# MECLabTUDA/Lifelong-nnUNet

Hardware: AMD Instinct MI355X
Metric: 3D patches/sec (whole node) + mean Dice vs ref, 5-level 3D Generic_UNet training step (higher is better)
Workload: dtype f16 (fp32 accumulate, fp32 master weights); 1 GPU; BASELINE configs[1]: nnUNetTrainerSequential.run_iteration, 160x192x160 patches, batch 2/GPU, num_pool 5, base 32, 3 logits; global_batch=2, parallelism=dp1, distinct_resident_batches=2, deterministic_wgrad=False

## Files before the change

lifelong-nnunet_amd/csrc/igemm_up2.hip:

```cpp
#include "igemm_common.h"

namespace {

constexpr int TZ = 2, TY = 8, TX = 8, PZ = 3, PY = 9, PX = 9;
constexpr int P = PZ * PY * PX;
constexpr int CK = 16, ROWB = 32, MB = 32;
constexpr int XBYTES = P * ROWB;
constexpr int XCHUNKS = P * 2;
constexpr int NT = 256;
constexpr int XN = (XCHUNKS + NT - 1) / NT;

template <int MODE>
struct UpCfg {
    static constexpr int NTAP = MODE == 0 ? 27 : 8;
    static constexpr int WBYTES = NTAP * MB * ROWB;
    static constexpr int WCHUNKS = NTAP * MB * 2;
    static constexpr int WN = (WCHUNKS + NT - 1) / NT;
};

__device__ __forceinline__ int up_xaddr(int pz, int py, int px, int c2) {
    return ((pz * PY + py) * PX + px) * ROWB + ((c2 ^ (py & 1)) << 4);
}
__device__ __forceinline__ int up_waddr(int row, int c2) { return row * ROWB + ((c2 ^ ((row >> 3) & 1)) << 4); }

__device__ __forceinline__ void up_lane_voxel(int v, int& r, int& x) {
    if (v < 4) { r = 0; x = v; }
    else if (v < 12) { r = 2; x = v - 4; }
    else if (v < 16) { r = 0; x = v - 8; }
    else if (v < 20) { r = 3; x = v - 16; }
    else if (v < 28) { r = 1; x = v - 20; }
    else { r = 3; x = v - 24; }
}

template <int MODE>
__global__ __launch_bounds__(NT, 2) void igemm_up2_kernel(const ConvParams p, int mblocks) {
    using Cfg = UpCfg<MODE>;
    constexpr int WN = Cfg::WN, WBYTES = Cfg::WBYTES, WCHUNKS = Cfg::WCHUNKS;
    extern __shared__ __attribute__((aligned(16))) char smem[];
    char* const xb = smem;
    char* const wb = smem + 2 * XBYTES;

    const int tid = threadIdx.x, lane = tid & 63, wave = tid >> 6;
    const int v = lane & 31, hk = lane >> 5;
    const int m0 = (blockIdx.x % mblocks) * MB;
    int t = blockIdx.x / mblocks;
    const int tx = t % p.tiles_x; t /= p.tiles_x;
    const int ty = t % p.tiles_y; t /= p.tiles_y;
    const int tz = t % p.tiles_z; t /= p.tiles_z;
    const int n = t, qz0 = tz * TZ, qy0 = ty * TY, qx0 = tx * TX;
    const int nchunks = (p.C + CK - 1) / CK;
    const bool interior = qz0 + PZ <= p.Di && qy0 + PY <= p.Hi && qx0 + PX <= p.Wi && (p.C % CK) == 0;

    int xrel[XN], xlds[XN];
#pragma unroll
    for (int i = 0; i < XN; ++i) {
        const int idx = min(i * NT + tid, XCHUNKS - 1);
        const int pos = idx >> 1, c2 = idx & 1;
        const int px = pos % PX, py = (pos / PX) % PY, pz = pos / (PX * PY);
        xrel[i] = ((pz * p.Hi + py) * p.Wi + px) * p.ld_x + c2 * 8;
        xlds[i] = up_xaddr(pz, py, px, c2);
    }
    int wrel[WN], wlds[WN];
#pragma unroll
    for (int i = 0; i < WN; ++i) {
        const int idx = min(i * NT + tid, WCHUNKS - 1);
        const int c2 = idx & 1, row = idx >> 1, r = row % MB, tl = row / MB;
        wrel[i] = (tl * MB + r) * 16 + c2 * 8;
        wlds[i] = up_waddr(row, c2);
    }

    half8 xr[XN], wr[WN];
    unsigned xok = 0;
    const half8 zero8 = {0, 0, 0, 0, 0, 0, 0, 0};
    const long xbase = ((((long)n * p.Di + qz0) * p.Hi + qy0) * p.Wi + qx0) * p.ld_x;
    const int nck16 = p.KCpad >> 4;
    const half_t* const wbase = p.wp + (long)(m0 >> 5) * nck16 * Cfg::NTAP * 512;

    auto load_x = [&](int c0) {
        if (interior) {
            const half_t* bp = p.x + xbase + c0;
#pragma unroll
            for (int i = 0; i < XN; ++i) xr[i] = *reinterpret_cast<const half8*>(bp + xrel[i]);
            xok = 0xFFFFu;
        } else {
            unsigned m = 0;
#pragma unroll
            for (int i = 0; i < XN; ++i) {
                const int idx = min(i * NT + tid, XCHUNKS - 1);
                const int pos = idx >> 1, c2 = idx & 1;
                const int px = pos % PX, py = (pos / PX) % PY, pz = pos / (PX * PY);
                const bool ok = qz0 + pz < p.Di && qy0 + py < p.Hi && qx0 + px < p.Wi && c0 + c2 * 8 < p.C;
                xr[i] = *reinterpret_cast<const half8*>(p.x + (ok ? xbase + c0 + xrel[i] : 0));
                m |= (ok ? 1u : 0u) << i;
            }
            xok = m;
        }
    };
    auto store_x = [&](char* buf) {
#pragma unroll
        for (int i = 0; i < XN; ++i)
            if (i * NT + tid < XCHUNKS) *reinterpret_cast<half8*>(buf + xlds[i]) = ((xok >> i) & 1u) ? xr[i] : zero8;
    };
    auto load_w = [&](int c0) {
#pragma unroll
        for (int i = 0; i < WN; ++i) wr[i] = *reinterpret_cast<const half8*>(wbase + (long)(c0 >> 4) * Cfg::NTAP * 512 + wrel[i]);
    };
    auto store_w = [&](char* buf) {
#pragma unroll
        for (int i = 0; i < WN; ++i)
            if (i * NT + tid < WCHUNKS) *reinterpret_cast<half8*>(buf + wlds[i]) = wr[i];
    };

    int vr, vx;
    up_lane_voxel(v, vr, vx);
    const int wz = wave >> 1, wy = (wave & 1) * 4 + vr;
    int lterm[2];
#pragma unroll
    for (int par = 0; par < 2; ++par) lterm[par] = ((wz * PY + wy) * PX + vx) * ROWB + ((hk ^ ((wy + par) & 1)) << 4);
    const int a_lane = v * ROWB + ((hk ^ ((v >> 3) & 1)) << 4);

    floatx16 acc[8];
#pragma unroll
    for (int c = 0; c < 8; ++c)
#pragma unroll
        for (int i = 0; i < 16; ++i) acc[c][i] = 0.f;

    load_x(0);
    load_w(0);
    store_x(xb);
    store_w(wb);
    __syncthreads();

#pragma unroll 1
    for (int ch = 0; ch < nchunks; ++ch) {
        const bool more = ch + 1 < nchunks;
        const char* xl = xb + (ch & 1) * XBYTES;
        const char* wl = wb + (ch & 1) * WBYTES;
        if (more) {
            load_x((ch + 1) * CK);
            load_w((ch + 1) * CK);
        }
        if (MODE == 0) {
            half8 fb[2][2][2];
#pragma unroll
            for (int oz = 0; oz < 2; ++oz)
#pragma unroll
                for (int oy = 0; oy < 2; ++oy)
#pragma unroll
                    for (int ox = 0; ox < 2; ++ox)
                        fb[oz][oy][ox] = *reinterpret_cast<const half8*>(xl + ((oz * PY + oy) * PX + ox) * ROWB + lterm[oy]);
#pragma unroll
            for (int cls = 0; cls < 8; ++cls) {
                const int pz = cls >> 2, py = (cls >> 1) & 1, px = cls & 1;
#pragma unroll
                for (int a = 0; a <= pz; ++a)
#pragma unroll
                    for (int b = 0; b <= py; ++b)
#pragma unroll
                        for (int c = 0; c <= px; ++c) {
                            const int dz = pz ? 2 * a : 1, dy = py ? 2 * b : 1, dx = px ? 2 * c : 1;
                            const int oz = pz ? 1 - a : 0, oy = py ? 1 - b : 0, ox = px ? 1 - c : 0;
                            const int slot = dz * 9 + dy * 3 + dx;
                            const half8 fa = *reinterpret_cast<const half8*>(wl + slot * MB * ROWB + a_lane);
                            acc[cls] = __builtin_amdgcn_mfma_f32_32x32x16_f16(fa, fb[oz][oy][ox], acc[cls], 0, 0, 0);
                        }
            }
        } else {
            const half8 fb = *reinterpret_cast<const half8*>(xl + lterm[0]);
#pragma unroll
            for (int cls = 0; cls < 8; ++cls) {
                const half8 fa = *reinterpret_cast<const half8*>(wl + cls * MB * ROWB + a_lane);
                acc[cls] = __builtin_amdgcn_mfma_f32_32x32x16_f16(fa, fb, acc[cls], 0, 0, 0);
            }
        }
        if (more) {
            store_x(xb + ((ch + 1) & 1) * XBYTES);
            store_w(wb + ((ch + 1) & 1) * WBYTES);
        }
        __syncthreads();
    }

    constexpr int RS = 1040;
    char* const stg = smem;
    const int qz = qz0 + wz, qy = qy0 + wy;
    const int skey = (vx >> 1) & 3;
    const int eox = (lane >> 2) & 15, ec = lane & 3;
    const int egx = 2 * qx0 + eox, em = m0 + ec * 8;
    auto out_ptr = [&](int pz, int rr) -> half8* {
        const int row = wave * 8 + rr, zl = row >> 4, oyl = row & 15;
        const int oz = 2 * (qz0 + zl) + pz, oy = 2 * qy0 + oyl;
        const bool ok = oz < p.Do && oy < p.Ho && egx < p.Wo && em < p.M;
        return ok ? reinterpret_cast<half8*>(p.y + ((((long)n * p.Do + oz) * p.Ho + oy) * p.Wo + egx) * p.ld_y + em) : nullptr;
    };
#pragma unroll
    for (int pz = 0; pz < 2; ++pz) {
        half8 olds[8];
        if (p.accumulate) {
#pragma unroll
            for (int rr = 0; rr < 8; ++rr) {
                const half8* d = out_ptr(pz, rr);
                olds[rr] = *(d ? d : reinterpret_cast<const half8*>(p.y));
            }
        }
#pragma unroll
        for (int c4 = 0; c4 < 4; ++c4) {
            const int cls = pz * 4 + c4, py = c4 >> 1, px = c4 & 1;
            char* vb = stg + (wz * 16 + 2 * wy + py) * RS + (2 * vx + px) * 64;
#pragma unroll
            for (int qq = 0; qq < 4; ++qq) {
                const half4 o = {(half_t)acc[cls][qq * 4 + 0], (half_t)acc[cls][qq * 4 + 1], (half_t)acc[cls][qq * 4 + 2],
                                 (half_t)acc[cls][qq * 4 + 3]};
                *reinterpret_cast<half4*>(vb + (((2 * qq + hk) ^ skey) << 3)) = o;
            }
        }
        __syncthreads();
        {
            const int rkey = (eox >> 2) & 3;
#pragma unroll
            for (int rr = 0; rr < 8; ++rr) {
                const int row = wave * 8 + rr;
                half8 v = *reinterpret_cast<const half8*>(stg + row * RS + eox * 64 + ((ec ^ (rkey >> 1)) << 4));
                if (rkey & 1) v = half8{v[4], v[5], v[6], v[7], v[0], v[1], v[2], v[3]};
                half8* dst = out_ptr(pz, rr);
                if (dst) {
                    if (p.accumulate) {
#pragma unroll
                        for (int e = 0; e < 8; ++e) v[e] = (half_t)((float)v[e] + (float)olds[rr][e]);
                    }
                    *dst = v;
                }
            }
        }
        if (pz == 0) __syncthreads();
    }
    (void)qz; (void)qy;
}

template <int MODE>
int launch_up2(hipStream_t s, ConvParams& p, const char* name) {
    using Cfg = UpCfg<MODE>;
    p.tiles_z = lnn_cdiv((p.Do + 1) / 2, TZ); p.tiles_y = lnn_cdiv((p.Ho + 1) / 2, TY); p.tiles_x = lnn_cdiv((p.Wo + 1) / 2, TX);
    const int mblocks = lnn_cdiv(p.M, MB);
    const long blocks = (long)p.N * p.tiles_z * p.tiles_y * p.tiles_x * mblocks;
    const size_t lds_main = 2 * XBYTES + 2 * Cfg::WBYTES, lds_stage = 32 * 1040;
    const size_t lds = lds_main > lds_stage ? lds_main : lds_stage;
    auto kern = igemm_up2_kernel<MODE>;
    static bool attr_set = false;
    if (!attr_set) {
        hipFuncSetAttribute(reinterpret_cast<const void*>(kern), hipFuncAttributeMaxDynamicSharedMemorySize, 80 * 1024);
        attr_set = true;
    }
    hipLaunchKernelGGL(kern, dim3((unsigned)blocks), dim3(NT), lds, s, p, mblocks);
    LNN_CHECK_LAUNCH(name);
    return LNN_OK;
}

}

int lnn_launch_up2_dgrad(hipStream_t s, ConvParams& p, const char* name) { return launch_up2<0>(s, p, name); }
int lnn_launch_up2_convT(hipStream_t s, ConvParams& p, const char* name) { return launch_up2<1>(s, p, name); }
```

lifelong-nnunet_amd/csrc/lnn_debug.h:

```cpp
#ifndef LNN_DEBUG_H
#define LNN_DEBUG_H
#include "../../include/lnn_hip.h"
#ifdef __cplusplus
extern "C" {
#endif

int lnn_debug_tr16_probe(lnn_stream_t s, float* out256);

int lnn_debug_set_phase_buffer(void* dev_ptr_6x_u64);
int lnn_debug_force_conv_kernel(int which);
int lnn_debug_force_down2_kernel(int which);
int lnn_debug_set_v9_zseg(int segments);

int lnn_debug_set_k133_v9(int mode);
int lnn_debug_last_k133_on_v9(void);

int lnn_debug_set_gen_mode(int mode);

int lnn_debug_last_dgrad_reduce_fused(void);

int lnn_debug_set_cu_budget(int cus);

#ifdef __cplusplus
}
#endif
#endif
```

lifelong-nnunet_amd/native.py:

```python
from __future__ import annotations

import ctypes as C
import os

_HERE = os.path.dirname(os.path.abspath(__file__))
LIB_PATH = os.environ.get("LNN_LIB_PATH") or os.path.join(_HERE, "csrc", "liblnn_hip.so")

_p = C.c_void_p
_i = C.c_int
_l = C.c_long
_f = C.c_float
_sz = C.c_size_t

SIGNATURES = {
    "lnn_last_error": (C.c_char_p, []),
    "lnn_version": (_i, []),
    "lnn_device_info": (_i, [C.POINTER(_i), C.POINTER(_i), C.c_char_p, _i]),
    "lnn_pack_weights": (_i, [_p, _p, _p, _i, _i, _i, _l, _l, _l]),
    "lnn_packed_weight_elems": (_sz, [_i, _i, _i]),
    "lnn_conv3d_fwd": (_i, [_p, _p, _i, _p, _p, _p, _i, _i, _i, _i, _i, _i, _i, _i]),
    "lnn_conv3d_dgrad": (_i, [_p, _p, _i, _p, _p, _i, _i, _i, _i, _i, _i, _i, _i, _i]),
    "lnn_conv3d_wgrad": (_i, [_p, _p, _i, _p, _i, _p, _i, _i, _i, _i, _i, _i, _i]),
    "lnn_conv3d_fwd_cat": (_i, [_p, _p, _p, _i, _i, _p, _p, _p, _i, _i, _i, _i, _i, _i, _i]),
    "lnn_conv3d_fwd_in_stats": (_i, [_p, _p, _p, _i, _i, _p, _p, _p, _i, _i, _i, _i, _i, _i, _i, _f, _p, _p, _p, _p, _l]),
    "lnn_conv3d_dgrad_ws": (_i, [_p, _p, _i, _p, _p, _i, _i, _i, _i, _i, _i, _i, _i, _i, _p, _l]),
    "lnn_conv3d_dgrad_cat": (_i, [_p, _p, _i, _p, _p, _p, _i, _i, _i, _i, _i, _i, _i, _i, _i]),
    "lnn_conv3d_dgrad_cat_ws": (_i, [_p, _p, _i, _p, _p, _p, _i, _i, _i, _i, _i, _i, _i, _i, _i, _p, _l]),
    "lnn_conv3d_wgrad_cat": (_i, [_p, _p, _p, _i, _i, _p, _i, _p, _i, _i, _i, _i, _i, _i]),
    "lnn_convT3d_k2s2_fwd": (_i, [_p, _p, _i, _p, _p, _i, _i, _i, _i, _i, _i, _i]),
    "lnn_convT3d_k2s2_dgrad": (_i, [_p, _p, _i, _p, _p, _i, _i, _i, _i, _i, _i, _i, _i]),
    "lnn_convT3d_k2s2_wgrad": (_i, [_p, _p, _i, _p, _i, _p, _i, _i, _i, _i, _i, _i]),
    "lnn_conv3d_wgrad_det": (_i, [_p, _p, _i, _p, _i, _p, _i, _i, _i, _i, _i, _i, _i, _p, _l]),
    "lnn_conv3d_wgrad_cat_det": (_i, [_p, _p, _p, _i, _i, _p, _i, _p, _i, _i, _i, _i, _i, _i, _p, _l]),
    "lnn_convT3d_k2s2_wgrad_det": (_i, [_p, _p, _i, _p, _i, _p, _i, _i, _i, _i, _i, _i, _p, _l]),
    "lnn_unpack_wgrad": (_i, [_p, _p, _p, _i, _i, _i, _l, _l, _l, _f, _i]),
    "lnn_pack_weights_batched": (_i, [_p, _p, _p, _p, _i, _l]),
    "lnn_unpack_wgrad_batched": (_i, [_p, _p, _p, _p, _i, _l, _f, _i]),
    "lnn_wgrad_panel_elems": (_sz, [_i, _i, _i]),
    "lnn_instnorm_stats": (_i, [_p, _p, _i, _l, _i, _f, _p, _p, _p]),
    "lnn_instnorm_lrelu_fwd": (_i, [_p, _p, _p, _i, _i, _l, _i, _p, _p, _p, _p, _f]),
    "lnn_instnorm_lrelu_seg_fwd": (_i, [_p, _p, _p, _i, _i, _l, _i, _p, _p, _p, _p, _f, _p, _p, _i]),
    "lnn_instnorm_lrelu_bwd": (_i, [_p, _p, _p, _i, _i, _l, _i, _p, _p, _p, _p, _f, _p, _p, _p, _f, _p]),
    "lnn_instnorm_ws_doubles": (_sz, [_i, _i]),
    "lnn_instnorm_lrelu_seg_bwd": (_i, [_p, _p, _p, _i, _p, _p, _p, _i, _i, _l, _i, _p, _p, _p, _p, _f, _p, _p, _f, _p]),
    "lnn_instnorm_lrelu_seg_bwd_ws_doubles": (_sz, [_i, _i]),
    "lnn_instnorm_lrelu_bwd_sums": (_i, [_p, _p, _p, _i, _i, _l, _i, _p, _p, _p, _p, _f, _p, _p, _f, _p]),
    "lnn_conv3d_dgrad_in_bwd_sums": (_i, [_p, _p, _i, _p, _p, _i, _i, _i, _i, _i, _i, _i, _p, _p, _p, _p, _p, _f, _p, _p, _f, _p, _p, _l]),
    "lnn_instnorm_lrelu_bwd_apply": (_i, [_p, _p, _p, _i, _i, _l, _i, _p, _p, _p, _p, _f, _p]),
    "lnn_instnorm_small_volume": (_i, []),
    "lnn_conv3d_fwd_in_lrelu": (_i, [_p, _p, _p, _i, _i, _p, _p, _p, _i, _i, _i, _i, _i, _i, _i, _f, _p, _p, _p, _p, _f, _p, _i, _p, _p, _l]),
    "lnn_conv3d_dgrad_in_bwd": (_i, [_p, _p, _i, _p, _p, _i, _i, _i, _i, _i, _i, _i, _p, _p, _p, _p, _p, _f, _p, _p, _f, _p, _p, _l]),
    "lnn_conv3d_wgrad_c1_in_bwd": (_i, [_p, _p, _p, _p, _i, _p, _i, _i, _i, _i, _i, _p, _p, _p, _p, _f, _p, _p, _l]),
    "lnn_seg1x1_fwd": (_i, [_p, _p, _i, _p, _p, _i, _l, _i, _i]),
    "lnn_seg1x1_bwd": (_i, [_p, _p, _i, _p, _p, _p, _i, _p, _i, _l, _i, _i, _i, _f, _p]),
    "lnn_seg1x1_bwd_ws_floats": (_sz, [_i, _i]),
    "lnn_dice_ce_fwd": (_i, [_p, _p, _p, _i, _i, _l, _i, _f, _p, _p]),
    "lnn_dice_ce_fwd_ds": (_i, [_p, _p, _p, _i, _i, _l, _i, _f, _p, _p, _f, _p, _i]),
    "lnn_dice_ce_bwd": (_i, [_p, _p, _p, _i, _i, _l, _i, _f, _p, _f, _p, _f, _p]),
    "lnn_dice_ce_loss_from_totals": (_i, [_p, _p, _i, _i, _l, _i, _f, _p]),
    "lnn_dice_ce_ws_doubles": (_sz, [_i, _i]),
    "lnn_online_dice_counts": (_i, [_p, _p, _p, _i, _i, _l, _p]),
    "lnn_kl_logits": (_i, [_p, _p, _p, _i, _i, _l, _f, _p, _p]),
    "lnn_kl_logits_ws_doubles": (_sz, [_i]),
    "lnn_plop_pseudo_labels": (_i, [_p, _p, _p, _p, _f, _i, _i, _i, _i, _i, _p, _p, _p, _p]),
    "lnn_local_pod": (_i, [_p, _p, _p, _i, _i, _i, _i, _i, _l, _l, _l, _l, _l, _i, _f, _i, _p, _p, _p]),
    "lnn_ewc_penalty_fwd": (_i, [_p, _p, _p, _p, _l, _f, _p, _p]),
    "lnn_ewc_penalty_bwd": (_i, [_p, _p, _p, _p, _l, _f, _f, _p, _p]),
    "lnn_fisher_square": (_i, [_p, _p, _p, _l, _f]),
    "lnn_fisher_accumulate": (_i, [_p, _p, _p, _l, _f, _f]),
    "lnn_fisher_ema": (_i, [_p, _p, _p, _l, _f, _f]),
    "lnn_rw_update": (_i, [_p, _p, _p, _p, _p, _p, _l, _f, _f, _p, _f, _f, _i]),
    "lnn_target_ce_fwd": (_i, [_p, _p, _p, _i, _i, _i, _l, _f, _i, _f, _p, _p]),
    "lnn_target_ce_bwd": (_i, [_p, _p, _p, _i, _i, _i, _l, _f, _i, _f, _p, _f, _p, _p]),
    "lnn_softmax_accumulate": (_i, [_p, _p, _p, _p, _p] + [_i] * 11 + [_f, _i]),
    "lnn_softmax_finalize": (_i, [_p, _p, _p, _i, _l, _p]),
    "lnn_gradnorm_sumsq": (_i, [_p, _p, _l, _f, _p, _i]),
    "lnn_flat_reduce_ws_doubles": (_sz, []),
    "lnn_sgd_nesterov_step_clipped": (_i, [_p, _p, _p, _p, _l, _f, _f, _f, _f, _f, _p]),
    "lnn_sgd_nesterov_step": (_i, [_p, _p, _p, _p, _l, _f, _f, _f, _f, _i]),
    "lnn_cast_f32_to_h": (_i, [_p, _p, _p, _l]),
    "lnn_f32_conv3d_fwd": (_i, [_p, _p, _i, _p, _p, _p, _i, _i, _i, _i, _i, _i, _i, _i]),
    "lnn_f32_conv3d_dgrad": (_i, [_p, _p, _i, _p, _p, _i, _i, _i, _i, _i, _i, _i, _i, _i]),
    "lnn_f32_conv3d_wgrad": (_i, [_p, _p, _i, _p, _i, _p, _i, _i, _i, _i, _i, _i, _i]),
    "lnn_f32_convT3d_k2s2_fwd": (_i, [_p, _p, _i, _p, _p, _i, _i, _i, _i, _i, _i, _i]),
    "lnn_f32_convT3d_k2s2_dgrad": (_i, [_p, _p, _i, _p, _p, _i, _i, _i, _i, _i, _i, _i, _i]),
    "lnn_f32_convT3d_k2s2_wgrad": (_i, [_p, _p, _i, _p, _i, _p, _i, _i, _i, _i, _i, _i]),
    "lnn_f32_conv3d_fwd_g": (_i, [_p, _p, _i, _p, _p, _p, _i] + [_i] * 12),
    "lnn_f32_conv3d_dgrad_g": (_i, [_p, _p, _i, _p, _p, _i] + [_i] * 13),
    "lnn_f32_conv3d_wgrad_g": (_i, [_p, _p, _i, _p, _i, _p] + [_i] * 12),
    "lnn_f32_convT3d_fwd_g": (_i, [_p, _p, _i, _p, _p, _i] + [_i] * 9),
    "lnn_f32_convT3d_dgrad_g": (_i, [_p, _p, _i, _p, _p, _i] + [_i] * 10),
    "lnn_f32_convT3d_wgrad_g": (_i, [_p, _p, _i, _p, _i, _p] + [_i] * 9),
    "lnn_image_to_cl_h": (_i, [_p, _p, _p, _i, _i, _l, _i]),
    "lnn_f32_image_to_cl": (_i, [_p, _p, _p, _i, _i, _l, _i]),
    "lnn_f32_instnorm_lrelu_fwd": (_i, [_p, _p, _i, _p, _i, _i, _l, _i, _f, _p, _p, _p, _p, _f]),
    "lnn_f32_instnorm_lrelu_bwd": (_i, [_p, _p, _i, _p, _i, _i, _l, _i, _p, _p, _p, _p, _f, _p, _p, _p]),
    "lnn_f32_seg1x1_fwd": (_i, [_p, _p, _i, _p, _p, _i, _l, _i, _i]),
    "lnn_f32_seg1x1_bwd": (_i, [_p, _p, _i, _p, _p, _p, _i, _p, _i, _l, _i, _i, _i]),
    "lnn_debug_tr16_probe": (_i, [_p, _p]),
    "lnn_debug_set_phase_buffer": (_i, [_p]),
    "lnn_debug_force_conv_kernel": (_i, [_i]),
    "lnn_debug_force_down2_kernel": (_i, [_i]),
    "lnn_debug_set_v9_zseg": (_i, [_i]),
    "lnn_debug_set_k133_v9": (_i, [_i]),
    "lnn_debug_last_k133_on_v9": (_i, []),
    "lnn_debug_set_gen_mode": (_i, [_i]),
    "lnn_debug_last_dgrad_reduce_fused": (_i, []),
    "lnn_debug_set_cu_budget": (_i, [_i]),
    "lnn_conv3d_fwd_g": (_i, [_p, _p, _i, _p, _p, _p, _i] + [_i] * 12 + [_p, _l]),
    "lnn_conv3d_dgrad_g": (_i, [_p, _p, _i, _p, _p, _i] + [_i] * 13 + [_p, _l]),
    "lnn_conv3d_wgrad_g": (_i, [_p, _p, _i, _p, _i, _p] + [_i] * 12 + [_p, _l]),
    "lnn_convT3d_fwd_g": (_i, [_p, _p, _i, _p, _p, _i] + [_i] * 9 + [_p, _l]),
    "lnn_convT3d_dgrad_g": (_i, [_p, _p, _i, _p, _p, _i] + [_i] * 10 + [_p, _l]),
    "lnn_convT3d_wgrad_g": (_i, [_p, _p, _i, _p, _i, _p] + [_i] * 9 + [_p, _l]),
    "lnn_convT3d_k2s2_fwd_ws": (_i, [_p, _p, _i, _p, _p, _i, _i, _i, _i, _i, _i, _i, _p, _l]),
    "lnn_convT3d_k2s2_dgrad_ws": (_i, [_p, _p, _i, _p, _p, _i, _i, _i, _i, _i, _i, _i, _i, _p, _l]),
}

_lib = None


class NativeLibraryMissing(RuntimeError):
    pass


def lib():
    global _lib
    if _lib is None:
        if not os.path.exists(LIB_PATH):
            raise NativeLibraryMissing(
                f"{LIB_PATH} not found: build it with `python -c 'import __graft_entry__ as g; g.build()'` "
                f"(make -C lifelong-nnunet_amd/csrc).  There is no CPU / PyTorch fallback.")
        h = C.CDLL(LIB_PATH)
        for name, (res, args) in SIGNATURES.items():
            fn = getattr(h, name)
            fn.restype = res
            fn.argtypes = args
        _lib = h
    return _lib


def _ptr(t):
    if t is None:
        return None
    return t.data_ptr() if hasattr(t, "data_ptr") else int(t)


def stream_handle():
    import torch
    return torch.cuda.current_stream().cuda_stream


_fn_cache = {}


def call(name, *args):
    fn = _fn_cache.get(name)
    if fn is None:
        fn = _fn_cache[name] = getattr(lib(), name)
    conv = []
    for a in args:
        c = a.__class__
        if c is int or c is float or a is None:
            conv.append(a)
        elif hasattr(a, "data_ptr"):
            conv.append(a.data_ptr())
        else:
            conv.append(a)
    rc = fn(stream_handle(), *conv)
    if rc != 0:
        raise RuntimeError(f"{name} failed ({rc}): {lib().lnn_last_error().decode()}")


def call_plain(name, *args):
    rc = getattr(lib(), name)(*args)
    if rc != 0:
        raise RuntimeError(f"{name} failed ({rc}): {lib().lnn_last_error().decode()}")


def query(name, *args):
    return getattr(lib(), name)(*args)


def device_info():
    cu, khz = C.c_int(0), C.c_int(0)
    buf = C.create_string_buffer(128)
    rc = lib().lnn_device_info(C.byref(cu), C.byref(khz), buf, 128)
    if rc != 0:
        raise RuntimeError(lib().lnn_last_error().decode())
    return {"cu_count": cu.value, "clock_khz": khz.value, "arch": buf.value.decode()}
```

Measured before the change: 104.8 patches/s.

## Add persistent streaming kernel for k2s2 transposed conv with resident weights

Adds a persistent transposed-conv (k2s2) kernel for C=64/128. Each block loads its full 32-row weight slice into LDS once, then loops over tiles assigned by group and stride, prefetching the next input tile into registers while the current one computes. The old kernel launched one block per tile and re-streamed weights per K chunk. The new path avoids that weight reload and launch overhead, at the cost of large LDS use (possibly one block per CU) and grid sizing tied to the CU count.

Result: no change. 104.8 patches/s, median of 5 (+0.0%).

```diff
diff --git a/lifelong-nnunet_amd/csrc/igemm_up2.hip b/lifelong-nnunet_amd/csrc/igemm_up2.hip
--- a/lifelong-nnunet_amd/csrc/igemm_up2.hip
+++ b/lifelong-nnunet_amd/csrc/igemm_up2.hip
@@ -236,10 +236,233 @@
     (void)qz; (void)qy;
 }
 
+template <int NCH>
+struct UpsCfg {
+    static constexpr int NTAP = UpCfg<1>::NTAP, WBYTES = UpCfg<1>::WBYTES;
+    static constexpr int CP = NCH * 2;
+    static constexpr int XPIECES = TZ * TY * TX * CP;
+    static constexpr int XN = (XPIECES + NT - 1) / NT;
+    static constexpr int XCH = TZ * PY * PX * ROWB;
+    static constexpr int WTOT = NCH * WBYTES, XTOT = NCH * XCH, STG = 32 * 1040;
+    static constexpr int LDS = WTOT + (XTOT > STG ? XTOT : STG);
+    static constexpr int BPC = 2 * LDS <= 160 * 1024 ? 2 : 1;
+    static constexpr int DEPTH = BPC == 2 ? 1 : 2;
+};
+
+__device__ __forceinline__ void up_lds_barrier() {
+    asm volatile("s_waitcnt lgkmcnt(0)" ::: "memory");
+    __builtin_amdgcn_s_barrier();
+    asm volatile("" ::: "memory");
+}
+
+template <int NCH>
+__global__ __launch_bounds__(NT, (UpsCfg<NCH>::BPC)) void igemm_up2_stream_kernel(const ConvParams p, int mblocks, int ngroups,
+                                                                                 int per_group) {
+    using Cfg = UpsCfg<NCH>;
+    constexpr int XN = Cfg::XN, XPIECES = Cfg::XPIECES, CP = Cfg::CP, DEPTH = Cfg::DEPTH;
+    static_assert(XPIECES % NT == 0, "every thread fetches XN pieces");
+    extern __shared__ __attribute__((aligned(16))) char smem[];
+    char* const wl = smem;
+    char* const xl = smem + Cfg::WTOT;
+    char* const stg = xl;
+
+    const int tid = threadIdx.x, lane = tid & 63, wave = tid >> 6;
+    const int v = lane & 31, hk = lane >> 5;
+    const int grp = blockIdx.x % ngroups;
+    int slot_in_grp = blockIdx.x / ngroups;
+    const int m0 = (slot_in_grp % mblocks) * MB;
+    slot_in_grp /= mblocks;
+    const int step = gridDim.x / (ngroups * mblocks);
+    const int total = p.N * p.tiles_z * p.tiles_y * p.tiles_x;
+    const int end = min((grp + 1) * per_group, total);
+    int it = grp * per_group + slot_in_grp;
+    if (it >= end) return;
+
+    {
+        const half_t* const wbase = p.wp + (long)(m0 >> 5) * Cfg::WTOT / 2;
+        for (int idx = tid; idx < Cfg::WTOT / 16; idx += NT)
+            *reinterpret_cast<half8*>(wl + up_waddr(idx >> 1, idx & 1)) = *reinterpret_cast<const half8*>(wbase + (long)idx * 8);
+    }
+
+    int n, qz0, qy0, qx0;
+    auto decode = [&](int item) {
+        int t = item;
+        qx0 = (t % p.tiles_x) * TX; t /= p.tiles_x;
+        qy0 = (t % p.tiles_y) * TY; t /= p.tiles_y;
+        qz0 = (t % p.tiles_z) * TZ; t /= p.tiles_z;
+        n = t;
+    };
+
+    half8 xr[DEPTH][XN];
+    unsigned xok[DEPTH] = {};
+    const half8 zero8 = {0, 0, 0, 0, 0, 0, 0, 0};
+    auto load_x = [&](int set) {
+        const long xbase = ((((long)n * p.Di + qz0) * p.Hi + qy0) * p.Wi + qx0) * p.ld_x;
+        unsigned m = 0;
+#pragma unroll
+        for (int i = 0; i < XN; ++i) {
+            const int idx = i * NT + tid;
+            const int pos = idx / CP, c8 = idx % CP;
+            const int px = pos % TX, py = (pos / TX) % TY, pz = pos / (TX * TY);
+            const bool ok = qz0 + pz < p.Di && qy0 + py < p.Hi && qx0 + px < p.Wi;
+            xr[set][i] = *reinterpret_cast<const half8*>(p.x + (ok ? xbase + ((pz * p.Hi + py) * p.Wi + px) * p.ld_x + c8 * 8 : 0));
+            m |= (ok ? 1u : 0u) << i;
+        }
+        xok[set] = m;
+    };
+    auto store_x = [&](int set) {
+#pragma unroll
+        for (int i = 0; i < XN; ++i) {
+            const int idx = i * NT + tid;
+            const int pos = idx / CP, c8 = idx % CP;
+            const int px = pos % TX, py = (pos / TX) % TY, pz = pos / (TX * TY);
+            *reinterpret_cast<half8*>(xl + (c8 >> 1) * Cfg::XCH + up_xaddr(pz, py, px, c8 & 1)) = ((xok[set] >> i) & 1u) ? xr[set][i] : zero8;
+        }
+    };
+
+    int vr, vx;
+    up_lane_voxel(v, vr, vx);
+    const int wz = wave >> 1, wy = (wave & 1) * 4 + vr;
+    const int lterm = ((wz * PY + wy) * PX + vx) * ROWB + ((hk ^ (wy & 1)) << 4);
+    const int a_lane = v * ROWB + ((hk ^ ((v >> 3) & 1)) << 4);
+    constexpr int RS = 1040;
+    const int skey = (vx >> 1) & 3;
+    const int eox = (lane >> 2) & 15, ec = lane & 3, em = m0 + ec * 8;
+    const int rkey = (eox >> 2) & 3;
+
+    auto do_item = [&](int set, int item) {
+        store_x(set);
+        up_lds_barrier();
+        if (item + DEPTH * step < end) {
+            decode(item + DEPTH * step);
+            load_x(set);
+        }
+        decode(item);
+        const int egx = 2 * qx0 + eox;
+        auto out_ptr = [&](int pz, int rr) -> half8* {
+            const int row = wave * 8 + rr, zl = row >> 4, oyl = row & 15;
+            const int oz = 2 * (qz0 + zl) + pz, oy = 2 * qy0 + oyl;
+            const bool ok = oz < p.Do && oy < p.Ho && egx < p.Wo && em < p.M;
+            return ok ? reinterpret_cast<half8*>(p.y + ((((long)n * p.Do + oz) * p.Ho + oy) * p.Wo + egx) * p.ld_y + em) : nullptr;
+        };
+
+        floatx16 acc[8];
+#pragma unroll
+        for (int c = 0; c < 8; ++c)
+#pragma unroll
+            for (int i = 0; i < 16; ++i) acc[c][i] = 0.f;
+
+#pragma unroll
+        for (int ch = 0; ch < NCH; ++ch) {
+            const half8 fb = *reinterpret_cast<const half8*>(xl + ch * Cfg::XCH + lterm);
+#pragma unroll
+            for (int cls = 0; cls < 8; ++cls) {
+                const half8 fa = *reinterpret_cast<const half8*>(wl + ch * Cfg::WBYTES + cls * MB * ROWB + a_lane);
+                acc[cls] = __builtin_amdgcn_mfma_f32_32x32x16_f16(fa, fb, acc[cls], 0, 0, 0);
+            }
+        }
+        up_lds_barrier();
+
+#pragma unroll
+        for (int pz = 0; pz < 2; ++pz) {
+#pragma unroll
+            for (int c4 = 0; c4 < 4; ++c4) {
+                const int cls = pz * 4 + c4, py = c4 >> 1, px = c4 & 1;
+                char* vb = stg + (wz * 16 + 2 * wy + py) * RS + (2 * vx + px) * 64;
+#pragma unroll
+                for (int qq = 0; qq < 4; ++qq) {
+                    const half4 o = {(half_t)acc[cls][qq * 4 + 0], (half_t)acc[cls][qq * 4 + 1], (half_t)acc[cls][qq * 4 + 2],
+                                     (half_t)acc[cls][qq * 4 + 3]};
+                    *reinterpret_cast<half4*>(vb + (((2 * qq + hk) ^ skey) << 3)) = o;
+                }
+            }
+            up_lds_barrier();
+#pragma unroll
+            for (int rr = 0; rr < 8; ++rr) {
+                const int row = wave * 8 + rr;
+                half8 o = *reinterpret_cast<const half8*>(stg + row * RS + eox * 64 + ((ec ^ (rkey >> 1)) << 4));
+                if (rkey & 1) o = half8{o[4], o[5], o[6], o[7], o[0], o[1], o[2], o[3]};
+                half8* dst = out_ptr(pz, rr);
+                if (dst) *dst = o;
+            }
+            up_lds_barrier();
+        }
+    };
+
+    decode(it);
+    load_x(0);
+    if (DEPTH == 2 && it + step < end) {
+        decode(it + step);
+        load_x(DEPTH - 1);
+    }
+#pragma unroll 1
+    for (; it < end; it += DEPTH * step) {
+        do_item(0, it);
+        if (DEPTH == 2 && it + step < end) do_item(DEPTH - 1, it + step);
+    }
+}
+
+int up2_num_cu() {
+    static int num_cu = 0;
+    if (!num_cu) {
+        int dev = 0;
+        hipDeviceProp_t prop;
+        num_cu = (hipGetDevice(&dev) == hipSuccess && hipGetDeviceProperties(&prop, dev) == hipSuccess) ? prop.multiProcessorCount : 256;
+    }
+    return lnn_cu_budget(num_cu);
+}
+
+int g_force_up2 = -1;
+int g_last_up2_streaming = 0;
+
+long up2_stream_lds_bytes(int mode, int C) {
+    const long ntap = mode == 0 ? 27 : 8, nch = C / CK;
+    const long w = ntap * MB * ROWB * nch, x = (mode == 0 ? PZ : TZ) * PY * PX * ROWB * nch, stg = 32 * 1040;
+    return w + (x > stg ? x : stg);
+}
+
+bool up2_streams(int mode, const ConvParams& p) {
+    if (g_force_up2 == 0) return false;
+    if (mode != 1 || p.accumulate) return false;
+    if (p.C != 64 && p.C != 128) return false;
+    if (p.KCpad != p.C || up2_stream_lds_bytes(mode, p.C) > 160 * 1024) return false;
+    return true;
+}
+
+template <int NCH>
+int launch_up2_stream(hipStream_t s, ConvParams& p, const char* name) {
+    using Cfg = UpsCfg<NCH>;
+    const int mblocks = lnn_cdiv(p.M, MB);
+    const long total = (long)p.N * p.tiles_z * p.tiles_y * p.tiles_x;
+    LNN_REQUIRE(total < (1L << 30), "%s: %ld tiles", name, total);
+    int G = Cfg::BPC * up2_num_cu() / mblocks;
+    if (G < 1) G = 1;
+    const int ngroups = G % 8 == 0 ? 8 : 1;
+    const int per_group = lnn_cdiv(total, ngroups);
+    int per_gm = G / ngroups;
+    if (per_gm > per_group) per_gm = per_group;
+    const int grid = ngroups * mblocks * per_gm;
+    auto kern = igemm_up2_stream_kernel<NCH>;
+    static bool attr_set = false;
+    if (!attr_set) {
+        const hipError_t e = hipFuncSetAttribute(reinterpret_cast<const void*>(kern), hipFuncAttributeMaxDynamicSharedMemorySize, Cfg::LDS);
+        if (e != hipSuccess) {
+            lnn_set_error("%s: %d bytes of dynamic LDS refused: %s", name, Cfg::LDS, hipGetErrorString(e));
+            return LNN_ERR_LAUNCH;
+        }
+        attr_set = true;
+    }
+    hipLaunchKernelGGL(kern, dim3((unsigned)grid), dim3(NT), Cfg::LDS, s, p, mblocks, ngroups, per_group);
+    LNN_CHECK_LAUNCH(name);
+    return LNN_OK;
+}
+
 template <int MODE>
 int launch_up2(hipStream_t s, ConvParams& p, const char* name) {
     using Cfg = UpCfg<MODE>;
     p.tiles_z = lnn_cdiv((p.Do + 1) / 2, TZ); p.tiles_y = lnn_cdiv((p.Ho + 1) / 2, TY); p.tiles_x = lnn_cdiv((p.Wo + 1) / 2, TX);
+    g_last_up2_streaming = up2_streams(MODE, p) ? 1 : 0;
+    if (g_last_up2_streaming) return p.C == 64 ? launch_up2_stream<4>(s, p, name) : launch_up2_stream<8>(s, p, name);
     const int mblocks = lnn_cdiv(p.M, MB);
     const long blocks = (long)p.N * p.tiles_z * p.tiles_y * p.tiles_x * mblocks;
     const size_t lds_main = 2 * XBYTES + 2 * Cfg::WBYTES, lds_stage = 32 * 1040;
@@ -247,7 +470,11 @@
     auto kern = igemm_up2_kernel<MODE>;
     static bool attr_set = false;
     if (!attr_set) {
-        hipFuncSetAttribute(reinterpret_cast<const void*>(kern), hipFuncAttributeMaxDynamicSharedMemorySize, 80 * 1024);
+        const hipError_t e = hipFuncSetAttribute(reinterpret_cast<const void*>(kern), hipFuncAttributeMaxDynamicSharedMemorySize, 80 * 1024);
+        if (e != hipSuccess) {
+            lnn_set_error("%s: 80 KB of dynamic LDS refused: %s", name, hipGetErrorString(e));
+            return LNN_ERR_LAUNCH;
+        }
         attr_set = true;
     }
     hipLaunchKernelGGL(kern, dim3((unsigned)blocks), dim3(NT), lds, s, p, mblocks);
@@ -257,5 +484,12 @@
 
 }
 
+extern "C" int lnn_debug_force_up2_kernel(int which) {
+    LNN_REQUIRE(which >= -1 && which <= 1, "lnn_debug_force_up2_kernel: %d is not one of -1, 0, 1", which);
+    g_force_up2 = which;
+    return LNN_OK;
+}
+extern "C" int lnn_debug_last_up2_streaming(void) { return g_last_up2_streaming; }
+
 int lnn_launch_up2_dgrad(hipStream_t s, ConvParams& p, const char* name) { return launch_up2<0>(s, p, name); }
 int lnn_launch_up2_convT(hipStream_t s, ConvParams& p, const char* name) { return launch_up2<1>(s, p, name); }
diff --git a/lifelong-nnunet_amd/csrc/lnn_debug.h b/lifelong-nnunet_amd/csrc/lnn_debug.h
--- a/lifelong-nnunet_amd/csrc/lnn_debug.h
+++ b/lifelong-nnunet_amd/csrc/lnn_debug.h
@@ -10,6 +10,8 @@
 int lnn_debug_set_phase_buffer(void* dev_ptr_6x_u64);
 int lnn_debug_force_conv_kernel(int which);
 int lnn_debug_force_down2_kernel(int which);
+int lnn_debug_force_up2_kernel(int which);
+int lnn_debug_last_up2_streaming(void);
 int lnn_debug_set_v9_zseg(int segments);
 
 int lnn_debug_set_k133_v9(int mode);
diff --git a/lifelong-nnunet_amd/native.py b/lifelong-nnunet_amd/native.py
--- a/lifelong-nnunet_amd/native.py
+++ b/lifelong-nnunet_amd/native.py
@@ -101,6 +101,8 @@
     "lnn_debug_set_phase_buffer": (_i, [_p]),
     "lnn_debug_force_conv_kernel": (_i, [_i]),
     "lnn_debug_force_down2_kernel": (_i, [_i]),
+    "lnn_debug_force_up2_kernel": (_i, [_i]),
+    "lnn_debug_last_up2_streaming": (_i, []),
     "lnn_debug_set_v9_zseg": (_i, [_i]),
     "lnn_debug_set_k133_v9": (_i, [_i]),
     "lnn_debug_last_k133_on_v9": (_i, []),
```
